# OpenwaterHealth/OpenLIFU-python

Measured on AMD Instinct MI355X. Metric: Mvoxel-elements/s pressure-field accumulate, higher is better.
Workload: dtype f32-acc/f16x2+e4m3-corr

## Files before the change

openlifu-python_amd/csrc/k_coset2.hip:

```cpp
#include <algorithm>
#include <cstdlib>
#include "k_types.hip.h"
#include "olx_ctx.h"
#include "olx_launch.h"

namespace olx {

constexpr int CP_TW = 14;
constexpr int CP_TROWS = 26, CP_ROW0 = 15;
constexpr int CP_PSZ = 364;
constexpr int CP_UW = 12;
constexpr int CP_SHARED = 4;
constexpr int CP_MT = 5;

#ifdef OLX_EXP_CUTRACE
static __device__ unsigned long long g_cutrace[16384][8][5];
#define OLX_CUTRACE(k, v) do { if (lane == 0 && blockIdx.y == 0 && blockIdx.x < 16384) g_cutrace[blockIdx.x][wave][k] = (v); } while (0)
#else
#define OLX_CUTRACE(k, v)
#endif

template <int MX, int MY, bool CLAMP, bool FP8, bool DIR = false, bool BOTH = true ,
          bool PONLY = false >
__global__ __launch_bounds__(COS_NW * 64, 4) void field_cosetp_k(
    const uint4* __restrict__ bfrag, float* __restrict__ pmag, float* __restrict__ inten,
    const int* __restrict__ targets ,
    const CosetBlock* __restrict__ blocks , const CosetParams P) {
    constexpr int NT = 2, THREADS = COS_NW * 64, PAIR = 2;
    static_assert(!(BOTH && PONLY), "one output or both");
    constexpr int TROWS = CP_TROWS, ROW0 = CP_ROW0, PSZ = CP_PSZ, MT = CP_MT;
    static_assert((PSZ / 2) % 2 == 0 && ((PSZ / 2) % 32 == 22 || (PSZ / 2) % 32 == 30), "16 planes on 16 distinct even 8-byte slots");
    constexpr int B_KS_U4 = 128;
    constexpr int B_BYTES = PAIR * 4 * NT * B_KS_U4 * 16;
    constexpr int T_WORDS = COS_ZB * PSZ;
    __shared__ __attribute__((aligned(16))) unsigned char smem[B_BYTES + T_WORDS * 4 + T_WORDS * 4 + 64];
    auto s_B = [&](int rec, int nt, int part) -> const uint4* { return reinterpret_cast<const uint4*>(smem) + ((size_t)(rec * NT + nt) * B_KS_U4 + part * 64); };
    unsigned* const s_hi = reinterpret_cast<unsigned*>(smem + B_BYTES);
    unsigned* const s_lo = s_hi + T_WORDS;
    const int tile = blockIdx.y;
    const int tid = threadIdx.x, lane = tid & 63, wave = __builtin_amdgcn_readfirstlane(tid >> 6);
    const int g = lane >> 4, p16 = lane & 15;
    OLX_CUTRACE(2, __builtin_readcyclecounter());
    OLX_CUTRACE(0, (unsigned long long)__builtin_amdgcn_s_getreg((31 << 11) | 4));
    OLX_CUTRACE(1, (unsigned long long)__builtin_amdgcn_s_getreg((31 << 11) | 20));
    const int item = blockIdx.x;
    {
    const CosetBlock BK = blocks[item];
    const int npos = BK.npos, KY = BK.KY, ky_magic = BK.ky_magic;
    if (npos <= 0) return;
    const int ibase = BK.ibase, jbase = BK.jbase;
    const int k0 = BK.k0;
    const int ntile = __builtin_amdgcn_readfirstlane((npos - wave + COS_NW - 1) / COS_NW);
    const int lane_off = p16 * PSZ - g * CP_TW;
    int toff[MT];
#pragma unroll
    for (int t = 0; t < MT; ++t) {
        const int pos = min(wave + COS_NW * t, npos - 1);
        const int kx = (pos * ky_magic) >> 16, ky = pos - kx * KY;
        toff[t] = (ky + ROW0) * CP_TW + (CP_UW - 8 - 2 * kx);
    }
    floatx4_t acc[MT][NT];
#pragma unroll
    for (int t = 0; t < MT; ++t)
#pragma unroll
        for (int nt = 0; nt < NT; ++nt) acc[t][nt] = floatx4_t{0.f, 0.f, 0.f, 0.f};
    const int nsbp = P.nsbp;
    const int n_sb = P.nsa * nsbp;
    bool reuse_ok = nsbp == PAIR;
#ifdef OLX_DEV_PINS
    reuse_ok = reuse_ok && P.cp_noreuse == 0;
#endif
    constexpr int CHUNK_U4 = PAIR * 4 * NT * B_KS_U4, PRE = CHUNK_U4 / THREADS;
    static_assert(CHUNK_U4 % THREADS == 0, "chunk must split evenly over the block");
    uint4 pre[PRE];
    const uint4* const bsrc = bfrag + (size_t)tile * n_sb * (4 * NT * B_KS_U4);
#pragma unroll
    for (int q = 0; q < PRE; ++q) {
        const int idx = tid + q * THREADS;
        pre[q] = idx < n_sb * 4 * NT * B_KS_U4 ? bsrc[idx] : make_uint4(0, 0, 0, 0);
    }
    OLX_STAMP(0);
    for (int sb0 = 0; sb0 < n_sb; sb0 += PAIR) {
        const int sa = sb0 / nsbp, sbb0 = sb0 - sa * nsbp;
        if (sb0 > 0) __syncthreads();
        const bool reuse = sb0 > 0 && reuse_ok;
        if (sb0 == 0) OLX_STAMP(1);
        if (sb0 == 2) OLX_STAMP(7);
        if constexpr (FP8) __builtin_amdgcn_s_setprio(1);
        if (k0 + wave * COS_P < P.nz) {
            int lane_o = lane;
            asm volatile("" : "+v"(lane_o));
            float dz2[COS_P];
#pragma unroll
            for (int z = 0; z < COS_P; ++z) {
                const float dz = (float)(k0 + wave * COS_P + z) * P.hz - P.flat_ez;
                dz2[z] = dz * dz;
            }
            auto entry = [&](const float r2, const float dz2v, const float dx, const float dy, const int o, const bool ok) __attribute__((always_inline)) {
                float d2 = r2 + dz2v;
                if (CLAMP) d2 = fmaxf(d2, P.dmin2);
                const float ri = __builtin_amdgcn_rsqf(d2);
                const float ph = d2 * ri;
                float rs = ri * P.g_scale;
                if constexpr (DIR) rs *= table_mod(dx, dy, ph, ri, P.dir_wx, P.dir_wy, P.absorb_l2);
                float gr = rs * __builtin_amdgcn_cosf(ph), gi = rs * __builtin_amdgcn_sinf(ph);
                asm volatile("" : "+v"(gr), "+v"(gi));
                half2_t hi;
                if constexpr (FP8) hi = __builtin_convertvector(float2_t{gr, gi}, half2_t);
                else hi = __builtin_bit_cast(half2_t, __builtin_amdgcn_cvt_pkrtz(gr, gi));
                float lr, li;
                const unsigned hw = __builtin_bit_cast(unsigned, hi);
                asm("v_fma_mix_f32 %0, %1, -1.0, %2 op_sel:[0,0,0] op_sel_hi:[1,0,0]" : "=v"(lr) : "v"(hw), "v"(gr));
                asm("v_fma_mix_f32 %0, %1, -1.0, %2 op_sel:[1,0,0] op_sel_hi:[1,0,0]" : "=v"(li) : "v"(hw), "v"(gi));
                unsigned lo_word;
                if constexpr (FP8) {
                    short2_t w;
                    w = __builtin_amdgcn_cvt_scalef32_pk_fp8_f32(w, lr, li, 1.0f / COS_F8_LO, false);
                    w = __builtin_amdgcn_cvt_scalef32_pk_fp8_f32(w, gr, gi, 1.0f / COS_F8_HI, true);
                    lo_word = __builtin_bit_cast(unsigned, w);
                } else {
                    lo_word = __builtin_bit_cast(unsigned, __builtin_amdgcn_cvt_pkrtz(lr, li));
                }
                if (ok && OLX_IN(o, T_WORDS, 0)) {
                    s_hi[o] = __builtin_bit_cast(unsigned, hi);
                    s_lo[o] = lo_word;
                }
            };
            auto fill = [&](auto reuse_c) __attribute__((always_inline)) {
                constexpr bool RU = decltype(reuse_c)::value != 0;
                constexpr int CW = RU ? CP_UW - CP_SHARED : CP_UW;
                constexpr int RPF = 64 / CW;
                constexpr int NRF = (TROWS - (RU ? COS_P : 1)) / RPF;
                static_assert(NRF * RPF == TROWS - (RU ? COS_P : 1) && (RU ? COS_P * COS_P : COS_P) <= RPF, "the tail rows fit one evaluation of the wave's planes");
                const int wl = lane_o / CW, ui = lane_o - CW * wl;
                const bool gen_lane = wl < RPF;
                const int Ulane = ibase + P.x_begin + P.ux0 + P.mx * (ui - 7);
                const int Wlane = jbase + P.uy0 + P.my * (wl - ROW0);
                const int tw_off = (wave * COS_P) * PSZ + wl * CP_TW + (CP_UW - 1 - ui);
                const float U = (float)(Ulane - 8 * P.mx * sa);
                const float dx = fmaf(U, P.hx_hi, fmaf(U, P.hx_lo, P.fx0));
                const float dx2 = dx * dx;
                const int Wsb = Wlane - 8 * P.my * sbb0;
#pragma unroll 2
                for (int r = 0; r < NRF; ++r) {
                    const float W = (float)(Wsb + RPF * P.my * r);
                    const float dy = fmaf(W, P.hy_hi, fmaf(W, P.hy_lo, P.fy0));
                    const float r2 = fmaf(dy, dy, dx2);
#pragma unroll
                    for (int z = 0; z < COS_P; ++z) entry(r2, dz2[z], dx, dy, z * PSZ + tw_off + RPF * r * CP_TW, gen_lane);
                }
                const bool last_row = KY + 14 >= TROWS - 1;
                if constexpr (RU) {
                    const int zt = wl >> 1, rowt = TROWS - COS_P + (wl & 1);
                    const float W = (float)(Wsb - P.my * wl + rowt * P.my);
                    const float dy = fmaf(W, P.hy_hi, fmaf(W, P.hy_lo, P.fy0));
                    float dzl = dz2[0];
#pragma unroll
                    for (int z = 1; z < COS_P; ++z) dzl = zt == z ? dz2[z] : dzl;
                    entry(fmaf(dy, dy, dx2), dzl, dx, dy, (wave * COS_P + zt) * PSZ + rowt * CP_TW + (CP_UW - 1 - ui), zt < COS_P && (last_row || rowt < TROWS - 1));
                } else if (last_row) {
                    const float W = (float)(Wsb - P.my * wl + (TROWS - 1) * P.my);
                    const float dy = fmaf(W, P.hy_hi, fmaf(W, P.hy_lo, P.fy0));
                    float dzl = dz2[0];
#pragma unroll
                    for (int z = 1; z < COS_P; ++z) dzl = wl == z ? dz2[z] : dzl;
                    entry(fmaf(dy, dy, dx2), dzl, dx, dy, (wave * COS_P + wl) * PSZ + (TROWS - 1) * CP_TW + (CP_UW - 1 - ui), wl < COS_P);
                }
            };
            if (reuse) {
                static_assert(COS_P * TROWS <= 64 && CP_UW - CP_SHARED == 8 && CP_TW % 2 == 0 && PSZ % 2 == 0, "one lane per (plane, row); aligned 8-byte moves");
                const int zm = lane_o >= TROWS ? 1 : 0;
                const int mo = (wave * COS_P + zm) * PSZ + (lane_o - zm * TROWS) * CP_TW;
                if (lane_o < COS_P * TROWS && OLX_IN(mo, T_WORDS - (CP_UW - 1), 3)) {
                    unsigned long long mv[4];
                    __builtin_memcpy(&mv[0], __builtin_assume_aligned(s_hi + mo + 8, 8), 8);
                    __builtin_memcpy(&mv[1], __builtin_assume_aligned(s_hi + mo + 10, 8), 8);
                    __builtin_memcpy(&mv[2], __builtin_assume_aligned(s_lo + mo + 8, 8), 8);
                    __builtin_memcpy(&mv[3], __builtin_assume_aligned(s_lo + mo + 10, 8), 8);
                    __builtin_memcpy(__builtin_assume_aligned(s_hi + mo, 8), &mv[0], 8);
                    __builtin_memcpy(__builtin_assume_aligned(s_hi + mo + 2, 8), &mv[1], 8);
                    __builtin_memcpy(__builtin_assume_aligned(s_lo + mo, 8), &mv[2], 8);
                    __builtin_memcpy(__builtin_assume_aligned(s_lo + mo + 2, 8), &mv[3], 8);
                }
                __builtin_amdgcn_fence(__ATOMIC_RELEASE, "wavefront");
                fill(IntC<1>{});
            } else {
                fill(IntC<0>{});
            }
        }
        if constexpr (FP8) __builtin_amdgcn_s_setprio(0);
#pragma unroll
        for (int q = 0; q < PRE; ++q) reinterpret_cast<uint4*>(smem)[tid + q * THREADS] = pre[q];
        if (sb0 == 0) OLX_STAMP(2);
        __syncthreads();
        if (sb0 == 0) OLX_STAMP(3);
        {
            const int nxt = (sb0 + PAIR) * 4 * NT * B_KS_U4, lim = n_sb * 4 * NT * B_KS_U4;
#pragma unroll
            for (int q = 0; q < PRE; ++q) {
                const int idx = nxt + tid + q * THREADS;
                if (idx < lim) pre[q] = bsrc[idx];
            }
        }
#pragma unroll
        for (int sl = 0; sl < PAIR; ++sl) {
            if (sbb0 + sl >= P.nsb) break;
            if constexpr (FP8) {
#pragma unroll
                for (int kb = 0; kb < 2; ++kb) {
                    Half8Bits bh[2][NT];
                    intx8_t b8[NT];
#pragma unroll
                    for (int nt = 0; nt < NT; ++nt) {
#pragma unroll
                        for (int ka = 0; ka < 2; ++ka) {
                            bh[ka][nt].u = s_B(sl * 4 + 2 * kb + ka, nt, 0)[lane];
                            const uint4 q = s_B(sl * 4 + 2 * kb + ka, nt, 1)[lane];
                            b8[nt][4 * ka + 0] = (int)q.x; b8[nt][4 * ka + 1] = (int)q.y; b8[nt][4 * ka + 2] = (int)q.z; b8[nt][4 * ka + 3] = (int)q.w;
                        }
                    }
#pragma unroll
                    for (int t = 0; t < MT; ++t) {
                        if (t >= ntile) continue;
                        Half8Bits ah[2];
                        intx8_t a8;
                        int lo_t = lane_off;
                        asm volatile("" : "+v"(lo_t));
                        const int ro = lo_t + toff[t];
#pragma unroll
                        for (int ka = 0; ka < 2; ++ka) {
                            const int kso = 4 * ka - (4 * kb + 8 * sl) * CP_TW;
                            if (!OLX_IN(ro + kso, T_WORDS - 3, 1)) continue;
                            const unsigned long long* ph2 = reinterpret_cast<const unsigned long long*>(s_hi + ro + kso);
                            const unsigned long long* pl2 = reinterpret_cast<const unsigned long long*>(s_lo + ro + kso);
                            const unsigned long long h0 = __hip_atomic_load(ph2, __ATOMIC_RELAXED, __HIP_MEMORY_SCOPE_WAVEFRONT);
                            const unsigned long long h1 = __hip_atomic_load(ph2 + 1, __ATOMIC_RELAXED, __HIP_MEMORY_SCOPE_WAVEFRONT);
                            const unsigned long long l0 = __hip_atomic_load(pl2, __ATOMIC_RELAXED, __HIP_MEMORY_SCOPE_WAVEFRONT);
                            const unsigned long long l1 = __hip_atomic_load(pl2 + 1, __ATOMIC_RELAXED, __HIP_MEMORY_SCOPE_WAVEFRONT);
                            ah[ka].w[0] = (unsigned)h0; ah[ka].w[1] = (unsigned)(h0 >> 32); ah[ka].w[2] = (unsigned)h1; ah[ka].w[3] = (unsigned)(h1 >> 32);
                            a8[4 * ka + 0] = (int)(unsigned)l0; a8[4 * ka + 1] = (int)(unsigned)(l0 >> 32);
                            a8[4 * ka + 2] = (int)(unsigned)l1; a8[4 * ka + 3] = (int)(unsigned)(l1 >> 32);
                        }
#pragma unroll
                        for (int nt = 0; nt < NT; ++nt) acc[t][nt] = __builtin_amdgcn_mfma_f32_16x16x32_f16(ah[0].h, bh[0][nt].h, acc[t][nt], 0, 0, 0);
#pragma unroll
                        for (int nt = 0; nt < NT; ++nt) acc[t][nt] = __builtin_amdgcn_mfma_f32_16x16x32_f16(ah[1].h, bh[1][nt].h, acc[t][nt], 0, 0, 0);
#pragma unroll
                        for (int nt = 0; nt < NT; ++nt)
                            acc[t][nt] = __builtin_amdgcn_mfma_scale_f32_16x16x128_f8f6f4(a8, b8[nt], acc[t][nt], 0, 0, 0, 128, 0, 127);
                    }
                }
            } else {
#pragma unroll
                for (int ks = 0; ks < 4; ++ks) {
                    const int ka = ks & 1, kb = ks >> 1;
                    Half8Bits bh[NT], bl[NT];
#pragma unroll
                    for (int nt = 0; nt < NT; ++nt) {
                        bh[nt].u = s_B(sl * 4 + ks, nt, 0)[lane];
                        bl[nt].u = s_B(sl * 4 + ks, nt, 1)[lane];
                    }
                    const int kso = 4 * ka - (4 * kb + 8 * sl) * CP_TW;
#pragma unroll
                    for (int t = 0; t < MT; ++t) {
                        if (t >= ntile) continue;
                        Half8Bits ah, al;
                        int lo_t = lane_off;
                        asm volatile("" : "+v"(lo_t));
                        const int ro = lo_t + toff[t];
                        if (!OLX_IN(ro + kso, T_WORDS - 3, 1)) continue;
                        const unsigned long long* ph2 = reinterpret_cast<const unsigned long long*>(s_hi + ro + kso);
                        const unsigned long long* pl2 = reinterpret_cast<const unsigned long long*>(s_lo + ro + kso);
                        const unsigned long long h0 = __hip_atomic_load(ph2, __ATOMIC_RELAXED, __HIP_MEMORY_SCOPE_WAVEFRONT);
                        const unsigned long long h1 = __hip_atomic_load(ph2 + 1, __ATOMIC_RELAXED, __HIP_MEMORY_SCOPE_WAVEFRONT);
                        const unsigned long long l0 = __hip_atomic_load(pl2, __ATOMIC_RELAXED, __HIP_MEMORY_SCOPE_WAVEFRONT);
                        const unsigned long long l1 = __hip_atomic_load(pl2 + 1, __ATOMIC_RELAXED, __HIP_MEMORY_SCOPE_WAVEFRONT);
                        ah.w[0] = (unsigned)h0; ah.w[1] = (unsigned)(h0 >> 32); ah.w[2] = (unsigned)h1; ah.w[3] = (unsigned)(h1 >> 32);
                        al.w[0] = (unsigned)l0; al.w[1] = (unsigned)(l0 >> 32); al.w[2] = (unsigned)l1; al.w[3] = (unsigned)(l1 >> 32);
#pragma unroll
                        for (int nt = 0; nt < NT; ++nt) acc[t][nt] = __builtin_amdgcn_mfma_f32_16x16x32_f16(ah.h, bh[nt].h, acc[t][nt], 0, 0, 0);
#pragma unroll
                        for (int nt = 0; nt < NT; ++nt) acc[t][nt] = __builtin_amdgcn_mfma_f32_16x16x32_f16(al.h, bh[nt].h, acc[t][nt], 0, 0, 0);
#pragma unroll
                        for (int nt = 0; nt < NT; ++nt) acc[t][nt] = __builtin_amdgcn_mfma_f32_16x16x32_f16(ah.h, bl[nt].h, acc[t][nt], 0, 0, 0);
                    }
                }
            }
        }
        if (sb0 == 0) OLX_STAMP(4);
    }
    OLX_STAMP(5);
    int lane_e = lane;
    asm volatile("" : "+v"(lane_e));
    const int c16 = lane_e >> 2;
    const int kz = k0 + 4 * (lane_e & 3);
    const int src_lane4 = (16 * (lane_e & 3) + (lane_e >> 2)) * 4;
    const float s_p = P.out_scale, s_i = P.out_scale * P.out_scale * P.inten_scale;
    const bool want_p = PONLY || (P.flags & 1u) != 0, want_i = !PONLY && (P.flags & 2u) != 0;
    constexpr int NOUT = PONLY ? 1 : NT;
#pragma unroll
    for (int t = 0; t < MT; ++t) {
        if (t >= ntile) continue;
        float o[NOUT][4];
#pragma unroll
        for (int r = 0; r < 4; r += 2) {
            const float2_t re = {acc[t][0][r], acc[t][0][r + 1]}, im = {acc[t][1][r], acc[t][1][r + 1]};
            const float2_t m = __builtin_elementwise_fma(re, re, im * im);
            o[0][r] = __builtin_amdgcn_sqrtf(m.x) * s_p;
            o[0][r + 1] = __builtin_amdgcn_sqrtf(m.y) * s_p;
            if constexpr (!PONLY) {
                const float2_t in = m * float2_t{s_i, s_i};
                o[1][r] = in.x;
                o[1][r + 1] = in.y;
            }
        }
#pragma unroll
        for (int nt = 0; nt < NOUT; ++nt) {
            floatx4_t v;
            v[0] = __builtin_bit_cast(float, __builtin_amdgcn_ds_bpermute(src_lane4, __builtin_bit_cast(int, o[nt][0])));
            v[1] = __builtin_bit_cast(float, __builtin_amdgcn_ds_bpermute(src_lane4, __builtin_bit_cast(int, o[nt][1])));
            v[2] = __builtin_bit_cast(float, __builtin_amdgcn_ds_bpermute(src_lane4, __builtin_bit_cast(int, o[nt][2])));
            v[3] = __builtin_bit_cast(float, __builtin_amdgcn_ds_bpermute(src_lane4, __builtin_bit_cast(int, o[nt][3])));
            acc[t][nt] = v;
        }
    }
    if (kz < P.nz) {
    const int4 tq = *reinterpret_cast<const int4*>(targets + ((size_t)tile * (MFMA_COLS * MFMA_MAX_NT) + c16) * 4);
    const int xm = P.nx - 1, ym = P.ny - 1;
    const int sxz = P.ny * P.nz;
    auto readout = [&](auto full_c) {
        constexpr bool FULL4 = decltype(full_c)::value != 0;
#pragma unroll
        for (int q = 0; q < 4; ++q) {
            const int code = q == 0 ? tq.x : q == 1 ? tq.y : q == 2 ? tq.z : tq.w;
            if (code < 0) continue;
            const unsigned m = (unsigned)code & 3u;
            const bool fx = (MX == 2) && (m & 1u), fy = (MY == 2) && ((MX == 2) ? (m >> 1) : (m & 1u));
            unsigned fxm = fx ? 0xFFFFFFFFu : 0u, fym = fy ? 0xFFFFFFFFu : 0u;
            asm volatile("" : "+v"(fxm), "+v"(fym));
            const long long fb = (long long)(code >> 2) * P.vox + kz;
            float* const base_p = pmag + fb;
// ... 82 lines not shown
```

openlifu-python_amd/csrc/olx.hip:

```cpp
#include "olx_ctx.h"

#include <dlfcn.h>
#include <unistd.h>

#include <algorithm>
#include <climits>
#include <cmath>
#include <cstring>
#include <thread>

#include "k_small.hip.h"
#include "olx_launch.h"
#include "olx_plan.h"
#include "k_toep.hip.h"

OLX_BOUNDS_READER(small)

template <class T> static int upload_if_changed(olx_ctx* c, DevBuf<T>& d, std::vector<T>& held, const std::vector<T>& v) {
    if (d.capacity() < v.size() || !d) held.clear();
    { int rc = d.reserve(c, v.size()); if (rc) return rc; }
    if (held.size() == v.size() && (v.empty() || !memcmp(held.data(), v.data(), sizeof(T) * v.size()))) return OLX_OK;
    HIPCHK(c, hipMemcpyAsync(d, v.data(), sizeof(T) * v.size(), hipMemcpyHostToDevice, c->stream));
    HIPCHK(c, hipStreamSynchronize(c->stream));
    held = v;
// ... 634 lines not shown
        MfmaParams& M = c->mp;
        M.nx = P.nx; M.ny = P.ny; M.nz = P.nz; M.n_el_pad = n_pad; M.x_begin = P.x_begin; M.n_tiles = ntiles;
        M.hx = P.hx; M.hy = P.hy; M.hz = P.hz; M.dmin2 = P.dmin2; M.flat_ez = P.flat_ez; M.flat_kz = P.flat_kz; M.flat_fz = P.flat_fz;
        M.g_scale = (float)sg; M.out_scale = (float)(1.0 / (sg * sw)); M.inten_scale = P.inten_scale;
        M.vox = P.vox; M.flags = P.flags;
        c->mfma_wscale = c->p0_pa / lambda * rev * sw;
        if (c->use_lattice) {
            const olx_ctx::Lattice& A = c->lat;
            LatParams& L = c->lp;
            c->lat_mt = 4;
            L.nx = P.nx; L.ny = P.ny; L.nz = P.nz;
            L.x_lo = c->mx == 2 ? P.nx / 2 : 0; L.y_lo = c->my == 2 ? P.ny / 2 : 0; L.x_begin = P.x_begin;
            L.mx = A.mx; L.my = A.my;
            L.tiles_x = ((P.nx - L.x_lo + 4 * A.mx - 1) / (4 * A.mx)) * 2 * A.mx;
            L.tiles_y = ((P.ny - L.y_lo + 4 * A.my - 1) / (4 * A.my)) * A.my;
            L.kgroups = (P.nz + 2 * c->lat_mt - 1) / (2 * c->lat_mt);
            L.nsa = A.nsa; L.nsb = A.nsb; L.nsbp = A.nsbp;
            const double offx = c->grid.origin[0] - A.x0, offy = c->grid.origin[1] - A.y0;
            L.ux0 = (int)std::llround(offx / c->grid.spacing[0]); L.uy0 = (int)std::llround(offy / c->grid.spacing[1]);
            L.fx0 = (float)((offx - L.ux0 * c->grid.spacing[0]) * rev); L.fy0 = (float)((offy - L.uy0 * c->grid.spacing[1]) * rev);
            const double hxw = c->grid.spacing[0] * rev, hyw = c->grid.spacing[1] * rev;
            L.hx_hi = (float)hxw; L.hx_lo = (float)(hxw - (double)L.hx_hi);
            L.hy_hi = (float)hyw; L.hy_lo = (float)(hyw - (double)L.hy_hi);
            L.hz = P.hz; L.dmin2 = P.dmin2; L.flat_ez = P.flat_ez;
            L.g_scale = M.g_scale; L.out_scale = M.out_scale; L.inten_scale = P.inten_scale;
            L.vox = P.vox; L.flags = P.flags;
            const long long tiles16 = coset_tiles16(P.nx - L.x_lo, P.ny - L.y_lo, A.mx, A.my, c->nt);
            c->fp8corr = fp8_want && c->use_coset && cos_fp8(c->nt) && !c->modifier();
            if (c->use_coset) {
                CosetParams& Q = c->cp;
                Q.nx = L.nx; Q.ny = L.ny; Q.nz = L.nz; Q.x_lo = L.x_lo; Q.y_lo = L.y_lo; Q.x_begin = L.x_begin; Q.mx = L.mx; Q.my = L.my;
                const int zb = COS_ZB;
                Q.xs = c->use_toep ? 1 : 2;
                olxplan::ToepPlan tp{};
                c->toep_nm = 1;
                int kyw = COS_KYW;
                if (c->use_toep) {
                    int saw_pin = 0, nm_pin = 0;
#ifdef OLX_DEV_PINS
                    if (const char* e = getenv("OLX_EXP_TOEP_SAW")) { const int v = atoi(e); if (v >= 8 && v <= 24) saw_pin = v; }
                    if (const char* e = getenv("OLX_EXP_TOEP_NM")) nm_pin = atoi(e) == 3 ? 3 : 1;
#endif
                    tp = olxplan::toep_plan(A.ax, Q.mx, Q.my, Q.xs, Q.nx - Q.x_lo, Q.ny - Q.y_lo, Q.nz, c->dir_lattice, saw_pin, nm_pin);
                    c->toep_nm = tp.nm; kyw = tp.kyw;
                }
                const int kxw = c->use_toep ? 8 * c->toep_nm : cos_kxw(c->nt);
                olxplan::coset_partition(Q, kxw, zb, kyw);
                Q.nsa = L.nsa; Q.nsb = L.nsb; Q.nsbp = L.nsbp; Q.ux0 = L.ux0; Q.uy0 = L.uy0; Q.fx0 = L.fx0; Q.fy0 = L.fy0;
                Q.hx_hi = L.hx_hi; Q.hx_lo = L.hx_lo; Q.hy_hi = L.hy_hi; Q.hy_lo = L.hy_lo; Q.hz = L.hz;
                Q.dmin2 = L.dmin2; Q.flat_ez = L.flat_ez; Q.g_scale = L.g_scale; Q.out_scale = L.out_scale; Q.inten_scale = L.inten_scale;
                Q.vox = L.vox; Q.flags = L.flags; Q.n_foci = F;
#ifdef OLX_DEV_PINS
                { const char* e = getenv("OLX_EXP_CP_NOREUSE"); Q.cp_noreuse = (e && atoi(e) != 0) ? 1 : 0; }
#endif
                Q.dir_wx = (c->dir_lattice && c->directivity) ? (float)(0.5 * c->h_size[0] / lambda) : 0.f;
                Q.dir_wy = (c->dir_lattice && c->directivity) ? (float)(0.5 * c->h_size[1] / lambda) : 0.f;
                Q.absorb_l2 = c->dir_lattice ? (float)(c->absorb_np_m * lambda * 1.4426950408889634) : 0.f;
                {
                    const std::vector<int> jobs = olxplan::build_store_jobs(tiles, MFMA_MAX_NT, MFMA_COLS, COS_JOBS, (P.flags & OLX_OUT_PMAG) != 0, (P.flags & OLX_OUT_INTENSITY) != 0);
                    int rc = upload_if_changed(c, c->d_jobs, c->up_jobs, jobs);
                    if (rc) return rc;
                }
                {
                    auto pick_grp = [&](int kblocks) {
                        const unsigned long long nb = (unsigned long long)Q.xs * Q.mx * Q.my * Q.nsx * Q.nsy * kblocks;
                        for (int g2 = std::min(kblocks, 32); g2 >= 2; --g2) if (kblocks % g2 == 0 && nb % (8ull * g2) == 0) return (unsigned)g2;
                        return 1u;
                    };
                    const int kcut = c->fp8corr ? c->fp8_kcut : 0;
                    const int kb_near = kcut / zb, kb_far = Q.kblocks - kb_near;
                    unsigned kgrp = pick_grp(kb_far), kgrp_near = kb_near > 0 ? pick_grp(kb_near) : 0u;
#ifdef OLX_DEV_PINS
                    if (const char* e = getenv("OLX_EXP_KGRP")) { kgrp = (unsigned)std::max(1, atoi(e)); if (kb_near > 0) kgrp_near = kgrp; }
#endif
                    const int rec_key[16] = {Q.nx, Q.ny, Q.nz, Q.x_lo, Q.y_lo, Q.mx, Q.my, Q.nsx, Q.nsy, Q.kblocks, zb, (int)kgrp, c->use_cosetp ? 40 : 0, Q.xs, kcut, (int)kgrp_near};
                    std::vector<CosetBlock> blk;
                    if (!c->up_blocks.empty() && memcmp(c->up_blocks_key, rec_key, sizeof rec_key) == 0) blk = c->up_blocks;
                    else {
                        std::string why;
                        CosetParams Qf = Q; Qf.kblocks = kb_far;
                        if (!olxplan::build_coset_blocks(Qf, zb, kgrp, c->use_cosetp ? 40 : 0, blk, why))
                            return fail(c, OLX_ESTATE, "kernel 2g: %s", why.c_str());
                        for (CosetBlock& b : blk) b.k0 += kcut;
                        if (kb_near > 0) {
                            std::vector<CosetBlock> near;
                            CosetParams Qn = Q; Qn.kblocks = kb_near;
                            if (!olxplan::build_coset_blocks(Qn, zb, kgrp_near, c->use_cosetp ? 40 : 0, near, why))
                                return fail(c, OLX_ESTATE, "kernel 2g: %s", why.c_str());
                            blk.insert(blk.end(), near.begin(), near.end());
                        }
                    }
                    const unsigned nblk = (unsigned)blk.size();
                    c->cp_nfar = nblk - (unsigned)((unsigned long long)Q.xs * Q.mx * Q.my * Q.nsx * Q.nsy * kb_near);
                    { int rc = upload_if_changed(c, c->d_cpblocks, c->up_blocks, blk); if (rc) return rc; }
                    memcpy(c->up_blocks_key, rec_key, sizeof rec_key);
                    c->cp_nblocks = nblk;
                }
                const double far_frac = c->fp8corr ? (double)std::max(0, P.nz - c->fp8_kcut) / (double)P.nz : 0.0;
                const double corr_units = 3.0 - far_frac;
                const std::string f8tag = !c->fp8corr ? "" : (c->fp8_kcut > 0 ? ",fp8corr from plane " + std::to_string(c->fp8_kcut) : ",fp8corr");
                const long long n_dense = (long long)((double)(P.nx - L.x_lo) * (P.ny - L.y_lo) * P.nz * (double)n * total_cols * 4.0 / 8192.0 * corr_units);
                if (c->use_toep) {
                    c->toep_saw = tp.saw;
                    c->toep_nsa = tp.nsa;
                    if (c->toep_nsa > 16) return fail(c, OLX_ESTATE, "kernel 2f: more than 16 super-block columns");
                    c->toep_ksmask = tp.ks_mask;
                    const int ksteps_total = tp.ksteps_total, e4_units = tp.e4_units;
                    for (int q = 0; q < 4; ++q) c->toep_targets[q] = tiles[0][0].tgt[q];
                    { int rc = c->d_cell.reserve(c, A.cell.size()); if (rc) return rc; }
                    HIPCHK(c, hipMemcpy(c->d_cell, A.cell.data(), sizeof(int) * A.cell.size(), hipMemcpyHostToDevice));
                    c->afrag_half = (size_t)ntiles * c->toep_nsa * 8 * A.nsb * 4 * 64;
                    { int rc = c->d_afrag.reserve(c, 2 * c->afrag_half); if (rc) return rc; }
                    long long n_mfma = 0;
                    const int wx = P.nx - L.x_lo, wy = P.ny - L.y_lo;
                    const double units_e4m3 = c->toep_nm == 2 ? 3.0 : (double)ksteps_total + (double)e4_units;
                    const double per_row = far_frac * units_e4m3 + (1.0 - far_frac) * 3.0 * ksteps_total;
                    for (int rx = 0; rx < Q.xs * A.mx; ++rx)
                        for (int ry = 0; ry < A.my; ++ry) {
                            const int kxa = rx < wx ? (wx - 1 - rx) / (Q.xs * A.mx) + 1 : 0, kya = ry < wy ? (wy - 1 - ry) / A.my + 1 : 0;
                            for (int sx = 0; sx < Q.nsx; ++sx)
                                for (int sy = 0; sy < Q.nsy; ++sy) {
                                    const int KX = (sx + 1) * kxa / Q.nsx - sx * kxa / Q.nsx, KY = (sy + 1) * kya / Q.nsy - sy * kya / Q.nsy;
                                    if (KX > 0 && KY > 0) n_mfma += (long long)((double)KY * per_row * (c->toep_nm > 1 ? 8 * c->toep_nm : 8) * A.nsb * Q.kblocks);
                                }
                        }
                    snprintf(nmbuf, sizeof nmbuf, "field_toep%s_k<mx%d,my%d,flat,%s%s> %d columns for %d foci x %d images in %d tile(s); "
                             "%dx%d lattice, pitch %dx%d voxels, %lld MFMA/launch (%lld dense), %d row tile(s) x %d y positions per block", "", c->mx, c->my, lat_clamp ? "clamp" : "noclamp", f8tag.c_str(),
                             total_cols, F, n_img, ntiles, A.ax, A.ay, A.mx, A.my, n_mfma, n_dense, c->toep_nm, kyw);
                } else {
                long long n_mfma = (long long)((double)tiles16 * ((P.nz + COS_P - 1) / COS_P) * A.nsa * A.nsb * 4 * c->nt * corr_units * ntiles);
                if (c->use_cosetp) {
                    long long npos_all = 0;
                    const int wx = P.nx - L.x_lo, wy = P.ny - L.y_lo;
                    for (int rx = 0; rx < 2 * A.mx; ++rx)
                        for (int ry = 0; ry < A.my; ++ry)
                            npos_all += (long long)(rx < wx ? (wx - 1 - rx) / (2 * A.mx) + 1 : 0) * (ry < wy ? (wy - 1 - ry) / A.my + 1 : 0);
                    n_mfma = (long long)((double)npos_all * Q.kblocks * A.nsa * A.nsb * 4 * c->nt * corr_units * ntiles);
                }
#ifdef OLX_DEV_PINS
                const char* const noreuse_tag = (c->use_cosetp && Q.cp_noreuse) ? ",noreuse" : "";
#else
                const char* const noreuse_tag = "";
#endif
                snprintf(nmbuf, sizeof nmbuf, "field_coset%s_k<nt%d,mx%d,my%d,flat,%s%s%s> %d columns for %d foci x %d images in %d tile(s); "
                         "%dx%d lattice, pitch %dx%d voxels, %lld MFMA/launch (%lld dense)", c->use_cosetp ? "p" : "", c->nt, c->mx, c->my, lat_clamp ? "clamp" : "noclamp",
                         f8tag.c_str(), noreuse_tag, total_cols, F, n_img, ntiles, A.ax, A.ay, A.mx, A.my, n_mfma, n_dense);
                }
            } else {
                const long long n_mfma = (long long)L.tiles_x * L.tiles_y * L.kgroups * A.nsa * A.nsb * 4 * c->lat_mt * c->nt * 3 * ntiles;
                snprintf(nmbuf, sizeof nmbuf, "field_lattice_k<mt%d,nt%d,mx%d,my%d,flat,%s> %d columns for %d foci x %d images in %d tile(s); "
                         "%dx%d lattice, pitch %dx%d voxels, %lld MFMA/launch", c->lat_mt, c->nt, c->mx, c->my, lat_clamp ? "clamp" : "noclamp",
                         total_cols, F, n_img, ntiles, A.ax, A.ay, A.mx, A.my, n_mfma);
            }
        } else {
            snprintf(nmbuf, sizeof nmbuf, "field_mfma_k<mt%d,nt%d,mx%d,my%d,%s,%s> %d columns for %d foci x %d images in %d tile(s)",
                     P.nz >= 48 ? 4 : 1, c->nt, c->mx, c->my, c->flat ? "flat" : "general", c->clamp ? "clamp" : (c->near ? "near" : "noclamp"), total_cols, F,
                     n_img, ntiles);
        }
    } else if (c->mx * c->my * c->nf == 1) {
        if (c->modifier()) snprintf(nmbuf, sizeof nmbuf, "field_accum_dir_k<4,%s> (%s%s%s)", c->clamp ? "clamp" : "noclamp", c->directivity ? "piston directivity" : "",
                                    (c->directivity && c->absorb_np_m > 0) ? ", " : "", c->absorb_np_m > 0 ? "uniform absorption" : "");
        else snprintf(nmbuf, sizeof nmbuf, "field_accum_k<4,%s,%s>", c->flat ? "flat" : "general", c->clamp ? "clamp" : (c->near ? "near" : "noclamp"));
    } else {
        const std::vector<int> perm = olxplan::mirror_perms(n, nm, c->dx == 2, c->dy == 2, c->h_px.data(), c->h_py.data(), nm);
        int rc = upload_if_changed(c, c->d_perm, c->up_perm, perm);
        if (!rc) rc = c->d_tab.reserve(c, (size_t)((F + c->nf - 1) / c->nf) * n * (SH_HEAD + 2 * nm * c->nf));
        if (rc) return rc;
        snprintf(nmbuf, sizeof nmbuf, "field_shared_k<4,mx%d,my%d,dx%d,dy%d,nf%d,%s,%s>", c->mx, c->my, c->dx, c->dy, c->nf,
                 c->flat ? "flat" : "general", c->clamp ? "clamp" : (c->near ? "near" : "noclamp"));
    }
    if (c->modifier() && c->use_mfma && !(c->use_lattice && c->use_coset)) {
        c->dir_lattice = false; c->allow_shared = false;
        return configure_variant_impl(c);
    }
    if (c->directivity && c->use_mfma) strncat(nmbuf, " +piston directivity in the tables", sizeof nmbuf - strlen(nmbuf) - 1);
    if (c->absorb_np_m > 0 && c->use_mfma) strncat(nmbuf, " +uniform absorption in the tables", sizeof nmbuf - strlen(nmbuf) - 1);
    c->variant = nmbuf;
    return OLX_OK;
}

static LatticePart lattice_part(const olx_ctx* c, bool below) {
    if (below) return {c->d_bfrag + c->bfrag_half, c->d_afrag + c->afrag_half, c->d_cpblocks + c->cp_nfar, c->cp_nblocks - c->cp_nfar, false};
    const bool split = c->fp8corr && c->cp_nfar < c->cp_nblocks;
    return {c->d_bfrag, c->d_afrag, c->d_cpblocks, split ? c->cp_nfar : c->cp_nblocks, c->fp8corr};
}

static int pack_if_needed(olx_ctx* c) {
    if (c->packed_version == c->steer_version) return OLX_OK;
    if (c->configured_version != c->steer_version) { int rc = configure_variant(c); if (rc) return rc; }
    const double lambda = c->c / c->freq;
    if (c->hetero) {
        olx_pack_hetero(c);
    } else if (c->use_mfma) {
        const double ox = c->mx == 2 ? c->grid.origin[0] + 0.5 * (c->grid.n[0] - 1) * c->grid.spacing[0] : c->grid.origin[0];
        const double oy = c->my == 2 ? c->grid.origin[1] + 0.5 * (c->grid.n[1] - 1) * c->grid.spacing[1] : c->grid.origin[1];
        dim3 g(c->mp.n_el_pad / 16, c->mp.n_tiles, c->nt);
        hipLaunchKernelGGL(mfma_pack_k, g, dim3(64), 0, c->stream, c->d_pos, c->d_area, c->n_el, c->mp.n_el_pad, c->d_delays,
                           c->d_apod, c->d_perm, ox, oy, c->grid.origin[2], c->freq, c->mfma_wscale, c->freq / c->c,
                           c->plan_foci, c->d_colinfo, c->use_lattice ? c->d_slot : nullptr,
// ... 71 lines not shown
    FieldParams& F = c->fp;
    F.nx = g->n[0]; F.ny = g->n[1]; F.nz = g->n[2]; F.n_el = c->n_el; F.x_begin = 0; F.vox = vox;
    F.flags = (flags & 3u) | OLX_OUT_PMAG; F.inten_scale = (float)(1e-4 / (2.0 * rho * cs));
    PulseParams& P = c->pulse;
    const double dt = c->pulse_dt;
    c->pulse_plan_dt = dt;
    P.n_el = c->n_el; P.n_foci = n_foci; P.n_t = c->pulse_nt; P.ny = g->n[1]; P.nz = g->n[2];
    P.ox = g->origin[0]; P.oy = g->origin[1]; P.oz = g->origin[2];
    P.hx = g->spacing[0]; P.hy = g->spacing[1]; P.hz = g->spacing[2];
    P.dmin = 0.5 * std::min({g->spacing[0], g->spacing[1], g->spacing[2]});
    P.inv_cdt = 1.0 / (cs * dt);
    P.tdt = c->pulse_cycles / (freq * dt);
    P.f0dt = freq * dt;
    P.dmin_f = (float)P.dmin; P.inv_cdt_f = (float)P.inv_cdt;
    P.absorb = (float)c->absorb_np_m;
    P.rot_c = (float)std::cos(2.0 * M_PI * P.f0dt); P.rot_s = (float)std::sin(2.0 * M_PI * P.f0dt);
    P.inten_scale = F.inten_scale;
    P.pii_scale = (float)(1e-4 * dt / (rho * cs));
    P.vox = vox;
    c->pulsed = true; c->pmax_live = false; c->agg_pmax_valid = false; c->pii_live = false;
    char nm[128];
    snprintf(nm, sizeof nm, "field_pulse_k (pulsed: %d samples, %.4g samples per burst)", c->pulse_nt, P.tdt);
    c->variant = nm;
    c->packed_version = ~0ull;
    c->planned = true; c->uploaded = false;
    return OLX_OK;
}

extern "C" {

int olx_field_plan(olx_ctx* c, const olx_grid* g, const olx_slab* slab, int n_foci, double freq, double cs,
                   double rho, double p0_pa, unsigned flags) {
    if (!c) return OLX_EINVAL;
    if (c->n_el <= 0) return fail(c, OLX_ESTATE, "olx_field_plan: call olx_set_elements first");
    if (c->n_foci <= 0) return fail(c, OLX_ESTATE, "olx_field_plan: no steering table (olx_bf_solve / olx_set_steering)");
    if (!g) return fail(c, OLX_EINVAL, "olx_field_plan: null grid");
    if (n_foci != c->n_foci) return fail(c, OLX_EINVAL, "olx_field_plan: n_foci %d != steering table foci %d", n_foci, c->n_foci);
    for (int a = 0; a < 3; ++a)
        if (g->n[a] < 1 || !(g->spacing[a] > 0)) return fail(c, OLX_EINVAL, "olx_field_plan: bad grid axis %d", a);
    if (!(freq > 0) || !(cs > 0) || !(rho > 0)) return fail(c, OLX_EINVAL, "olx_field_plan: freq, c, rho must be > 0");
    if (!(flags & (OLX_OUT_PMAG | OLX_OUT_INTENSITY | OLX_OUT_COMPLEX))) return fail(c, OLX_EINVAL, "olx_field_plan: no outputs selected");
    if (c->pulse_nt > 0) return plan_pulse(c, g, slab, n_foci, freq, cs, rho, p0_pa, flags);
    if (flags & OLX_OUT_PMAX) return fail(c, OLX_EINVAL, "olx_field_plan: OLX_OUT_PMAX needs a pulsed plan (olx_field_pulse)");
    if (flags & OLX_OUT_PII) return fail(c, OLX_EINVAL, "olx_field_plan: OLX_OUT_PII needs a pulsed plan (olx_field_pulse)");
    if (flags & ~(OLX_OUT_PMAG | OLX_OUT_INTENSITY | OLX_OUT_COMPLEX | OLX_FIELD_FP8_CORRECTION | OLX_FIELD_FP16_CORRECTION | OLX_FIELD_DIRECTIVITY)) return fail(c, OLX_EINVAL, "olx_field_plan: unknown flag bits 0x%x", flags);
    if ((flags & OLX_FIELD_DIRECTIVITY) && c->h_xaxis.size() != 3 * (size_t)c->n_el)
        return fail(c, OLX_ESTATE, "olx_field_plan: OLX_FIELD_DIRECTIVITY needs olx_set_element_apertures");
    olx_slab s{0, g->n[0]};
    if (slab) s = *slab;
    if (s.x_begin < 0 || s.x_count < 1 || s.x_begin + s.x_count > g->n[0]) return fail(c, OLX_EINVAL, "olx_field_plan: slab outside grid");
    HIPCHK(c, hipSetDevice(c->device));
    {
        std::string env;
        for (const char* name : {"OLX_FIELD_VARIANT", "OLX_FP8_CORRECTION", "OLX_EXP_TOEP_SAW", "OLX_EXP_TOEP_NM", "OLX_EXP_KGRP", "OLX_INTENSITY_STORED", "OLX_EXP_CP_NOREUSE"}) { const char* e = getenv(name); env += e ? e : ""; env += '|'; }
        const bool same = c->planned && !c->uploaded && !c->hetero && !c->pulsed && memcmp(&c->grid, g, sizeof *g) == 0 && c->slab.x_begin == s.x_begin &&
                          c->slab.x_count == s.x_count && c->plan_foci == n_foci && c->freq == freq && c->c == cs && c->rho == rho &&
                          c->p0_pa == p0_pa && c->flags == flags && c->plan_absorb == c->absorb_np_m && c->nbuf == (c->comm_active() ? olx_ctx::NBUF : 1) && c->plan_env == env;
        c->plan_env = env;
        if (same) {
            c->agg_local = -1; c->agg_total = 0;
            if (c->packed_version != c->steer_version) return configure_variant(c);
            return OLX_OK;
        }
    }
    HIPCHK(c, hipStreamSynchronize(c->stream));
    c->grid = *g; c->slab = s; c->plan_foci = n_foci; c->hetero = false;
    c->pulsed = false; c->pmax_live = false; c->agg_pmax_valid = false; c->pii_live = false;
    c->agg_local = -1; c->agg_total = 0;
    c->freq = freq; c->c = cs; c->rho = rho; c->p0_pa = p0_pa; c->flags = flags; c->plan_absorb = c->absorb_np_m;
    const long long vox = (long long)s.x_count * g->n[1] * g->n[2];
    pii_regrid(c, vox);
    const size_t total = (size_t)vox * n_foci;
    c->nbuf = c->comm_active() ? olx_ctx::NBUF : 1;
    { const char* pin = getenv("OLX_INTENSITY_STORED"); c->derive_i = (flags & OLX_OUT_INTENSITY) && !(pin && *pin && strcmp(pin, "0") != 0); }
    c->inten_live = false;
    { int rc = reserve_outputs(c, total, c->nbuf, (flags & OLX_OUT_INTENSITY) && !c->derive_i, (flags & OLX_OUT_COMPLEX) != 0, true); if (rc) return rc; }
    if (c->derive_i) c->d_inten.release();
    { int rc = c->d_tab.reserve(c, (size_t)n_foci * c->n_el * TAB_STRIDE); if (rc) return rc; }
    FieldParams& P = c->fp;
    P.nx = s.x_count; P.ny = g->n[1]; P.nz = g->n[2]; P.n_el = c->n_el;
    P.x_begin = s.x_begin;
    const double rev = freq / cs;
    P.hx = (float)(g->spacing[0] * rev); P.hy = (float)(g->spacing[1] * rev); P.hz = (float)(g->spacing[2] * rev);
    const double dmin = 0.5 * std::min({g->spacing[0], g->spacing[1], g->spacing[2]});
    P.dmin2 = (float)(dmin * dmin * rev * rev);
    P.inten_scale = (float)(1e-4 / (2.0 * rho * cs));
    P.vox = vox; P.flags = ((flags & 7u) | OLX_OUT_PMAG) & ~(c->derive_i ? (unsigned)OLX_OUT_INTENSITY : 0u);
    c->directivity = (flags & OLX_FIELD_DIRECTIVITY) != 0;
    const int n = c->n_el;
    const double* hz = c->h_pos.data() + 2 * (size_t)n;
    c->flat = true;
    for (int e = 1; e < n; ++e) if (hz[e] != hz[0]) { c->flat = false; break; }
    P.flat_ez = (float)((hz[0] - g->origin[2]) * rev);
    { const double kz = std::rint((hz[0] - g->origin[2]) / g->spacing[2]); P.flat_kz = (float)kz; P.flat_fz = (float)(((hz[0] - g->origin[2]) - kz * g->spacing[2]) * rev); }
    double lo[3], hi[3];
    for (int a = 0; a < 3; ++a) {
        const int b = (a == 0) ? s.x_begin : 0;
        const int cnt = (a == 0) ? s.x_count : g->n[a];
        lo[a] = g->origin[a] + b * g->spacing[a];
        hi[a] = g->origin[a] + (b + cnt - 1) * g->spacing[a];
    }
    c->clamp = false;
    const double guard = 2.0 * dmin;
    double min_d2 = 1e300;
    for (int e = 0; e < n; ++e) {
        double d2 = 0;
        for (int a = 0; a < 3; ++a) {
// ... 1992 lines not shown
```

openlifu-python_amd/csrc/olx_params.h:

```cpp
#pragma once
#ifdef __HIPCC__
#include <hip/hip_runtime.h>
#endif
#include <stdint.h>

namespace olx {

constexpr int BF_THREADS = 256;
constexpr int SH_HEAD = 8;
constexpr int TAB_STRIDE = 8;
constexpr int FIELD_THREADS = 256;

struct FieldParams {
    int nx, ny, nz;
    int n_el;
    int x_begin;
    float hx, hy, hz;
    float dmin2;
    float inten_scale;
    float flat_ez;
    float flat_kz, flat_fz;
    float absorb_l2;
    long long vox;
    unsigned flags;
// ... 16 lines not shown
struct MfmaParams {
    int nx, ny, nz, n_el_pad;
    int x_begin, n_tiles;
    float hx, hy, hz;
    float dmin2, flat_ez, g_scale;
    float flat_kz, flat_fz;
    float out_scale;
    float inten_scale;
    long long vox;
    unsigned flags;
};

struct LatParams {
    int nx, ny, nz;
    int x_lo, y_lo;
    int x_begin;
    int mx, my;
    int tiles_x, tiles_y;
    int kgroups;
    int nsa, nsb;
    int nsbp;
    int ux0, uy0;
    float fx0, fy0;
    float hx_hi, hx_lo, hy_hi, hy_lo, hz;
    float dmin2, flat_ez, g_scale, out_scale, inten_scale;
    long long vox;
    unsigned flags;
};

constexpr int LAT_ELEMS_LDS = 128;
constexpr int LAT_TW = 10;
constexpr int LAT_PSZ = 116;
constexpr int LAT_THREADS = 512;

struct CosetParams {
    int nx, ny, nz;
    int x_lo, y_lo, x_begin;
    int mx, my;
    int nsx, nsy;
    int xs;
    int kblocks;
    int nsa, nsb;
    int nsbp;
    int ux0, uy0;
    float fx0, fy0, hx_hi, hx_lo, hy_hi, hy_lo, hz;
    float dmin2, flat_ez, g_scale, out_scale, inten_scale;
    float dir_wx, dir_wy;
    float absorb_l2;
    long long vox;
    unsigned flags;
    int n_foci;
#ifdef OLX_DEV_PINS
    int cp_noreuse;
#endif
};

struct CosetBlock {
    int ibase, jbase;
    int k0;
    int npos;
    int KY;
    int ky_magic;
    int KX;
    int pad_;
};

constexpr int COS_NW = 8;
constexpr int COS_P = 2;
constexpr int COS_ZB = COS_NW * COS_P;
constexpr int COS_KYW = 11;
constexpr int COS_JOBS = 64;
constexpr int cos_kxw(int nt) { return nt >= 4 ? 2 : (nt >= 2 ? 3 : 6); }
constexpr bool cos_fp8(int nt) { return nt <= 2; }
constexpr float COS_F8_LO = 32.0f, COS_F8_HI = 1.0f / 64.0f;

constexpr int HET_TAB_HEAD = 12;

struct HeteroParams {
    int n_planes;
    int n_layers;
    int n_foci;
    float u0, v0;
    float inv_hx, inv_hy;
    int nxg, nyg;
    int xg_begin;
    float kappa;
};

struct PulseParams {
    int n_el, n_foci, n_t;
    int ny, nz;
    double ox, oy, oz, hx, hy, hz;
    double dmin;
    double inv_cdt;
    double tdt;
    double f0dt;
    float dmin_f, inv_cdt_f;
    float absorb;
    float rot_c, rot_s;
    float inten_scale;
    float pii_scale;
    long long vox;
};

struct ThermalParams {
    int nx, ny, nz;
// ... 57 lines not shown
```

Baseline: 113.9 million.

## Evaluate next reuse-fill entries ahead into registers during MFMA phase

For the FP8 coset kernel, the Green's-function entries for the next sub-block's reuse fill are computed into registers right after the barrier, before the MFMA loop, and only stored to LDS at the next iteration's fill. The goal is to overlap the transcendental-heavy fill with matrix work and shorten the time between barriers. The B-fragment prefetch is also moved to after the MFMA loop for this path. This adds 14 held registers per lane and changes load timing, which can raise register pressure under launch bounds of 4 blocks.

```diff
diff --git a/openlifu-python_amd/csrc/k_coset2.hip b/openlifu-python_amd/csrc/k_coset2.hip
--- a/openlifu-python_amd/csrc/k_coset2.hip
+++ b/openlifu-python_amd/csrc/k_coset2.hip
@@ -12,6 +12,7 @@
 constexpr int CP_UW = 12;
 constexpr int CP_SHARED = 4;
 constexpr int CP_MT = 5;
+constexpr int CP_AHEAD_N = 7;
 
 #ifdef OLX_EXP_CUTRACE
 static __device__ unsigned long long g_cutrace[16384][8][5];
@@ -27,6 +28,8 @@
     const int* __restrict__ targets ,
     const CosetBlock* __restrict__ blocks , const CosetParams P) {
     constexpr int NT = 2, THREADS = COS_NW * 64, PAIR = 2;
+    constexpr bool AHEAD = FP8;
+    constexpr bool PRE_LATE = AHEAD;
     static_assert(!(BOTH && PONLY), "one output or both");
     constexpr int TROWS = CP_TROWS, ROW0 = CP_ROW0, PSZ = CP_PSZ, MT = CP_MT;
     static_assert((PSZ / 2) % 2 == 0 && ((PSZ / 2) % 32 == 22 || (PSZ / 2) % 32 == 30), "16 planes on 16 distinct even 8-byte slots");
@@ -70,6 +73,90 @@
 #ifdef OLX_DEV_PINS
     reuse_ok = reuse_ok && P.cp_noreuse == 0;
 #endif
+    bool ahead_ok = AHEAD && reuse_ok;
+#ifdef OLX_DEV_PINS
+    ahead_ok = ahead_ok && P.cp_nofillahead == 0;
+#endif
+    const bool my_planes = k0 + wave * COS_P < P.nz;
+    unsigned held_hi[CP_AHEAD_N], held_lo[CP_AHEAD_N];
+    auto plane_dz2 = [&](const int z) __attribute__((always_inline)) {
+        const float dz = (float)(k0 + wave * COS_P + z) * P.hz - P.flat_ez;
+        float q = dz * dz;
+        if constexpr (AHEAD) asm volatile("" : "+v"(q));
+        return q;
+    };
+    auto entry = [&](const float r2, const float dz2v, const float dx, const float dy, unsigned& hi_word, unsigned& lo_word) __attribute__((always_inline)) {
+        float d2 = r2 + dz2v;
+        if (CLAMP) d2 = fmaxf(d2, P.dmin2);
+        const float ri = __builtin_amdgcn_rsqf(d2);
+        const float ph = d2 * ri;
+        float rs = ri * P.g_scale;
+        if constexpr (DIR) rs *= table_mod(dx, dy, ph, ri, P.dir_wx, P.dir_wy, P.absorb_l2);
+        float gr = rs * __builtin_amdgcn_cosf(ph), gi = rs * __builtin_amdgcn_sinf(ph);
+        asm volatile("" : "+v"(gr), "+v"(gi));
+        half2_t hi;
+        if constexpr (FP8) hi = __builtin_convertvector(float2_t{gr, gi}, half2_t);
+        else hi = __builtin_bit_cast(half2_t, __builtin_amdgcn_cvt_pkrtz(gr, gi));
+        float lr, li;
+        const unsigned hw = __builtin_bit_cast(unsigned, hi);
+        asm("v_fma_mix_f32 %0, %1, -1.0, %2 op_sel:[0,0,0] op_sel_hi:[1,0,0]" : "=v"(lr) : "v"(hw), "v"(gr));
+        asm("v_fma_mix_f32 %0, %1, -1.0, %2 op_sel:[1,0,0] op_sel_hi:[1,0,0]" : "=v"(li) : "v"(hw), "v"(gi));
+        if constexpr (FP8) {
+            short2_t w;
+            w = __builtin_amdgcn_cvt_scalef32_pk_fp8_f32(w, lr, li, 1.0f / COS_F8_LO, false);
+            w = __builtin_amdgcn_cvt_scalef32_pk_fp8_f32(w, gr, gi, 1.0f / COS_F8_HI, true);
+            lo_word = __builtin_bit_cast(unsigned, w);
+        } else {
+            lo_word = __builtin_bit_cast(unsigned, __builtin_amdgcn_cvt_pkrtz(lr, li));
+        }
+        hi_word = hw;
+    };
+    auto put = [&](const int o, const bool ok, const unsigned hi_word, const unsigned lo_word) __attribute__((always_inline)) {
+        if (ok && OLX_IN(o, T_WORDS, 0)) {
+            s_hi[o] = hi_word;
+            s_lo[o] = lo_word;
+        }
+    };
+    constexpr int RU_CW = CP_UW - CP_SHARED, RU_ROWS = 64 / RU_CW, RU_NR = (CP_TROWS - COS_P) / RU_ROWS;
+    static_assert(CP_AHEAD_N == RU_NR * COS_P + 1 && RU_CW == 8 && RU_ROWS == 8 && COS_P == 2, "the reuse form: 3 rounds x 2 planes and the tail rows");
+    auto ru_slot = [&](const int e, const int lane_o, int& o, bool& ok) __attribute__((always_inline)) {
+        const int wl = lane_o >> 3, ui = lane_o & 7;
+        if (e < RU_NR * COS_P) {
+            o = (wave * COS_P + (e & 1)) * PSZ + (wl + RU_ROWS * (e >> 1)) * CP_TW + (CP_UW - 1 - ui);
+            ok = true;
+        } else {
+            const int zt = wl >> 1, rowt = CP_TROWS - COS_P + (wl & 1);
+            o = (wave * COS_P + zt) * PSZ + rowt * CP_TW + (CP_UW - 1 - ui);
+            ok = zt < COS_P && (KY + 14 >= CP_TROWS - 1 || rowt < CP_TROWS - 1);
+        }
+    };
+    auto ru_eval_all = [&](const int sa_f, const int sbb_f, unsigned (&hi_words)[CP_AHEAD_N], unsigned (&lo_words)[CP_AHEAD_N]) __attribute__((always_inline)) {
+        int lane_o = lane;
+        asm volatile("" : "+v"(lane_o));
+        const int wl = lane_o >> 3, ui = lane_o & 7;
+        const float U = (float)(ibase + P.x_begin + P.ux0 + P.mx * (ui - 7) - 8 * P.mx * sa_f);
+        const float dx = fmaf(U, P.hx_hi, fmaf(U, P.hx_lo, P.fx0));
+        const float dx2 = dx * dx;
+        const int Wsb = jbase + P.uy0 + P.my * (wl - ROW0) - 8 * P.my * sbb_f;
+        float dz2[COS_P];
+#pragma unroll
+        for (int z = 0; z < COS_P; ++z) dz2[z] = plane_dz2(z);
+#pragma unroll
+        for (int r = 0; r < RU_NR; ++r) {
+            const float W = (float)(Wsb + RU_ROWS * P.my * r);
+            const float dy = fmaf(W, P.hy_hi, fmaf(W, P.hy_lo, P.fy0));
+            const float r2 = fmaf(dy, dy, dx2);
+#pragma unroll
+            for (int z = 0; z < COS_P; ++z) entry(r2, dz2[z], dx, dy, hi_words[COS_P * r + z], lo_words[COS_P * r + z]);
+        }
+        const int zt = wl >> 1, rowt = CP_TROWS - COS_P + (wl & 1);
+        const float W = (float)(Wsb - P.my * wl + rowt * P.my);
+        const float dy = fmaf(W, P.hy_hi, fmaf(W, P.hy_lo, P.fy0));
+        float dzl = dz2[0];
+#pragma unroll
+        for (int z = 1; z < COS_P; ++z) dzl = zt == z ? dz2[z] : dzl;
+        entry(fmaf(dy, dy, dx2), dzl, dx, dy, hi_words[CP_AHEAD_N - 1], lo_words[CP_AHEAD_N - 1]);
+    };
     constexpr int CHUNK_U4 = PAIR * 4 * NT * B_KS_U4, PRE = CHUNK_U4 / THREADS;
     static_assert(CHUNK_U4 % THREADS == 0, "chunk must split evenly over the block");
     uint4 pre[PRE];
@@ -87,44 +174,17 @@
         if (sb0 == 0) OLX_STAMP(1);
         if (sb0 == 2) OLX_STAMP(7);
         if constexpr (FP8) __builtin_amdgcn_s_setprio(1);
-        if (k0 + wave * COS_P < P.nz) {
+        const bool held = reuse && ahead_ok;
+        if (my_planes) {
             int lane_o = lane;
             asm volatile("" : "+v"(lane_o));
             float dz2[COS_P];
 #pragma unroll
-            for (int z = 0; z < COS_P; ++z) {
-                const float dz = (float)(k0 + wave * COS_P + z) * P.hz - P.flat_ez;
-                dz2[z] = dz * dz;
-            }
-            auto entry = [&](const float r2, const float dz2v, const float dx, const float dy, const int o, const bool ok) __attribute__((always_inline)) {
-                float d2 = r2 + dz2v;
-                if (CLAMP) d2 = fmaxf(d2, P.dmin2);
-                const float ri = __builtin_amdgcn_rsqf(d2);
-                const float ph = d2 * ri;
-                float rs = ri * P.g_scale;
-                if constexpr (DIR) rs *= table_mod(dx, dy, ph, ri, P.dir_wx, P.dir_wy, P.absorb_l2);
-                float gr = rs * __builtin_amdgcn_cosf(ph), gi = rs * __builtin_amdgcn_sinf(ph);
-                asm volatile("" : "+v"(gr), "+v"(gi));
-                half2_t hi;
-                if constexpr (FP8) hi = __builtin_convertvector(float2_t{gr, gi}, half2_t);
-                else hi = __builtin_bit_cast(half2_t, __builtin_amdgcn_cvt_pkrtz(gr, gi));
-                float lr, li;
-                const unsigned hw = __builtin_bit_cast(unsigned, hi);
-                asm("v_fma_mix_f32 %0, %1, -1.0, %2 op_sel:[0,0,0] op_sel_hi:[1,0,0]" : "=v"(lr) : "v"(hw), "v"(gr));
-                asm("v_fma_mix_f32 %0, %1, -1.0, %2 op_sel:[1,0,0] op_sel_hi:[1,0,0]" : "=v"(li) : "v"(hw), "v"(gi));
-                unsigned lo_word;
-                if constexpr (FP8) {
-                    short2_t w;
-                    w = __builtin_amdgcn_cvt_scalef32_pk_fp8_f32(w, lr, li, 1.0f / COS_F8_LO, false);
-                    w = __builtin_amdgcn_cvt_scalef32_pk_fp8_f32(w, gr, gi, 1.0f / COS_F8_HI, true);
-                    lo_word = __builtin_bit_cast(unsigned, w);
-                } else {
-                    lo_word = __builtin_bit_cast(unsigned, __builtin_amdgcn_cvt_pkrtz(lr, li));
-                }
-                if (ok && OLX_IN(o, T_WORDS, 0)) {
-                    s_hi[o] = __builtin_bit_cast(unsigned, hi);
-                    s_lo[o] = lo_word;
-                }
+            for (int z = 0; z < COS_P; ++z) dz2[z] = plane_dz2(z);
+            auto entry_put = [&](const float r2, const float dz2v, const float dx, const float dy, const int o, const bool ok) __attribute__((always_inline)) {
+                unsigned hw, lw;
+                entry(r2, dz2v, dx, dy, hw, lw);
+                put(o, ok, hw, lw);
             };
             auto fill = [&](auto reuse_c) __attribute__((always_inline)) {
                 constexpr bool RU = decltype(reuse_c)::value != 0;
@@ -147,7 +207,7 @@
                     const float dy = fmaf(W, P.hy_hi, fmaf(W, P.hy_lo, P.fy0));
                     const float r2 = fmaf(dy, dy, dx2);
 #pragma unroll
-                    for (int z = 0; z < COS_P; ++z) entry(r2, dz2[z], dx, dy, z * PSZ + tw_off + RPF * r * CP_TW, gen_lane);
+                    for (int z = 0; z < COS_P; ++z) entry_put(r2, dz2[z], dx, dy, z * PSZ + tw_off + RPF * r * CP_TW, gen_lane);
                 }
                 const bool last_row = KY + 14 >= TROWS - 1;
                 if constexpr (RU) {
@@ -157,14 +217,14 @@
                     float dzl = dz2[0];
 #pragma unroll
                     for (int z = 1; z < COS_P; ++z) dzl = zt == z ? dz2[z] : dzl;
-                    entry(fmaf(dy, dy, dx2), dzl, dx, dy, (wave * COS_P + zt) * PSZ + rowt * CP_TW + (CP_UW - 1 - ui), zt < COS_P && (last_row || rowt < TROWS - 1));
+                    entry_put(fmaf(dy, dy, dx2), dzl, dx, dy, (wave * COS_P + zt) * PSZ + rowt * CP_TW + (CP_UW - 1 - ui), zt < COS_P && (last_row || rowt < TROWS - 1));
                 } else if (last_row) {
                     const float W = (float)(Wsb - P.my * wl + (TROWS - 1) * P.my);
                     const float dy = fmaf(W, P.hy_hi, fmaf(W, P.hy_lo, P.fy0));
                     float dzl = dz2[0];
 #pragma unroll
                     for (int z = 1; z < COS_P; ++z) dzl = wl == z ? dz2[z] : dzl;
-                    entry(fmaf(dy, dy, dx2), dzl, dx, dy, (wave * COS_P + wl) * PSZ + (TROWS - 1) * CP_TW + (CP_UW - 1 - ui), wl < COS_P);
+                    entry_put(fmaf(dy, dy, dx2), dzl, dx, dy, (wave * COS_P + wl) * PSZ + (TROWS - 1) * CP_TW + (CP_UW - 1 - ui), wl < COS_P);
                 }
             };
             if (reuse) {
@@ -183,7 +243,17 @@
                     __builtin_memcpy(__builtin_assume_aligned(s_lo + mo + 2, 8), &mv[3], 8);
                 }
                 __builtin_amdgcn_fence(__ATOMIC_RELEASE, "wavefront");
-                fill(IntC<1>{});
+                if (held) {
+#pragma unroll
+                    for (int e = 0; e < CP_AHEAD_N; ++e) {
+                        int o;
+                        bool ok;
+                        ru_slot(e, lane_o, o, ok);
+                        put(o, ok, held_hi[e], held_lo[e]);
+                    }
+                } else {
+                    fill(IntC<1>{});
+                }
             } else {
                 fill(IntC<0>{});
             }
@@ -194,13 +264,20 @@
         if (sb0 == 0) OLX_STAMP(2);
         __syncthreads();
         if (sb0 == 0) OLX_STAMP(3);
-        {
+        auto request_next = [&]() __attribute__((always_inline)) {
+            int tid_o = tid;
+            if constexpr (PRE_LATE) asm volatile("" : "+v"(tid_o));
             const int nxt = (sb0 + PAIR) * 4 * NT * B_KS_U4, lim = n_sb * 4 * NT * B_KS_U4;
 #pragma unroll
             for (int q = 0; q < PRE; ++q) {
-                const int idx = nxt + tid + q * THREADS;
-                if (idx < lim) pre[q] = bsrc[idx];
+                const int idx = nxt + tid_o + q * THREADS;
+                if constexpr (PRE_LATE) pre[q] = idx < lim ? bsrc[idx] : make_uint4(0, 0, 0, 0);
+                else if (idx < lim) pre[q] = bsrc[idx];
             }
+        };
+        if constexpr (!PRE_LATE) request_next();
+        if constexpr (AHEAD) if (ahead_ok && my_planes && sb0 + PAIR < n_sb) {
+            ru_eval_all(sa + 1, sbb0, held_hi, held_lo);
         }
 #pragma unroll
         for (int sl = 0; sl < PAIR; ++sl) {
@@ -287,6 +364,7 @@
                 }
             }
         }
+        if constexpr (PRE_LATE) request_next();
         if (sb0 == 0) OLX_STAMP(4);
     }
     OLX_STAMP(5);
diff --git a/openlifu-python_amd/csrc/olx.hip b/openlifu-python_amd/csrc/olx.hip
--- a/openlifu-python_amd/csrc/olx.hip
+++ b/openlifu-python_amd/csrc/olx.hip
@@ -710,6 +710,7 @@
                 Q.vox = L.vox; Q.flags = L.flags; Q.n_foci = F;
 #ifdef OLX_DEV_PINS
                 { const char* e = getenv("OLX_EXP_CP_NOREUSE"); Q.cp_noreuse = (e && atoi(e) != 0) ? 1 : 0; }
+                { const char* e = getenv("OLX_EXP_CP_NOFILLAHEAD"); Q.cp_nofillahead = (e && atoi(e) != 0) ? 1 : 0; }
 #endif
                 Q.dir_wx = (c->dir_lattice && c->directivity) ? (float)(0.5 * c->h_size[0] / lambda) : 0.f;
                 Q.dir_wy = (c->dir_lattice && c->directivity) ? (float)(0.5 * c->h_size[1] / lambda) : 0.f;
@@ -796,13 +797,13 @@
                     n_mfma = (long long)((double)npos_all * Q.kblocks * A.nsa * A.nsb * 4 * c->nt * corr_units * ntiles);
                 }
 #ifdef OLX_DEV_PINS
-                const char* const noreuse_tag = (c->use_cosetp && Q.cp_noreuse) ? ",noreuse" : "";
+                const std::string pin_tags = std::string((c->use_cosetp && Q.cp_noreuse) ? ",noreuse" : "") + ((c->use_cosetp && Q.cp_nofillahead) ? ",nofillahead" : "");
 #else
-                const char* const noreuse_tag = "";
+                const std::string pin_tags;
 #endif
                 snprintf(nmbuf, sizeof nmbuf, "field_coset%s_k<nt%d,mx%d,my%d,flat,%s%s%s> %d columns for %d foci x %d images in %d tile(s); "
                          "%dx%d lattice, pitch %dx%d voxels, %lld MFMA/launch (%lld dense)", c->use_cosetp ? "p" : "", c->nt, c->mx, c->my, lat_clamp ? "clamp" : "noclamp",
-                         f8tag.c_str(), noreuse_tag, total_cols, F, n_img, ntiles, A.ax, A.ay, A.mx, A.my, n_mfma, n_dense);
+                         f8tag.c_str(), pin_tags.c_str(), total_cols, F, n_img, ntiles, A.ax, A.ay, A.mx, A.my, n_mfma, n_dense);
                 }
             } else {
                 const long long n_mfma = (long long)L.tiles_x * L.tiles_y * L.kgroups * A.nsa * A.nsb * 4 * c->lat_mt * c->nt * 3 * ntiles;
@@ -980,7 +981,7 @@
     HIPCHK(c, hipSetDevice(c->device));
     {
         std::string env;
-        for (const char* name : {"OLX_FIELD_VARIANT", "OLX_FP8_CORRECTION", "OLX_EXP_TOEP_SAW", "OLX_EXP_TOEP_NM", "OLX_EXP_KGRP", "OLX_INTENSITY_STORED", "OLX_EXP_CP_NOREUSE"}) { const char* e = getenv(name); env += e ? e : ""; env += '|'; }
+        for (const char* name : {"OLX_FIELD_VARIANT", "OLX_FP8_CORRECTION", "OLX_EXP_TOEP_SAW", "OLX_EXP_TOEP_NM", "OLX_EXP_KGRP", "OLX_INTENSITY_STORED", "OLX_EXP_CP_NOREUSE", "OLX_EXP_CP_NOFILLAHEAD"}) { const char* e = getenv(name); env += e ? e : ""; env += '|'; }
         const bool same = c->planned && !c->uploaded && !c->hetero && !c->pulsed && memcmp(&c->grid, g, sizeof *g) == 0 && c->slab.x_begin == s.x_begin &&
                           c->slab.x_count == s.x_count && c->plan_foci == n_foci && c->freq == freq && c->c == cs && c->rho == rho &&
                           c->p0_pa == p0_pa && c->flags == flags && c->plan_absorb == c->absorb_np_m && c->nbuf == (c->comm_active() ? olx_ctx::NBUF : 1) && c->plan_env == env;
diff --git a/openlifu-python_amd/csrc/olx_params.h b/openlifu-python_amd/csrc/olx_params.h
--- a/openlifu-python_amd/csrc/olx_params.h
+++ b/openlifu-python_amd/csrc/olx_params.h
@@ -92,6 +92,7 @@
     int n_foci;
 #ifdef OLX_DEV_PINS
     int cp_noreuse;
+    int cp_nofillahead;
 #endif
 };
 
```

Result: faster. 115.2 million (median of 6 runs) (+1.1%).
